# robotseu/ORB_Line_SLAM

Measured on AMD Instinct MI355X. Metric: stereo frames/s extract+match (ORB+LBD), KITTI 1242x375, higher is better.
Workload: dtype u8; 1 GPU; C3: 1242x375 stereo, 2000 ORB + 500 LBD per image, extract + stereo point/line match + f2f LBD match + SearchByBoW vs the previous frame (synthetic k=10 L=6 vocabulary, ComputeBoW included); parallelism=frame-sharded x1, distinct_pairs=512, order=shuffled, scene=default

## Files before the change

orb_line_slam_amd/csrc/api.cpp:

```cpp
#include "olf_internal.hpp"
#include "line_internal.hpp"
#include "../../include/orbline.h"
#include <map>
#include <mutex>
#include <cstring>
#include <mutex>

namespace olf {
static thread_local std::string g_err;
void set_error(const std::string& s) { g_err = s; }
}

using namespace olf;

struct olf_ctx {
    olf_params params;
    int W = 0, H = 0, max_images = 0;
    int device = 0;
    hipStream_t stream = nullptr;
    OrbHostTables orb;
    OrbDeviceBufs ob;
    uint8_t* d_images = nullptr;
    olf_keypoint* d_kps = nullptr;
    uint8_t* d_desc = nullptr;
// ... 183 lines not shown
    for (void* p : c->allocs) (void)hipFree(p);
    for (void* p : c->scratch) if (p) (void)hipFree(p);
    for (auto& r : c->prof_recs) { (void)hipEventDestroy(r.a); (void)hipEventDestroy(r.b); }
    for (hipEvent_t e : c->prof_pool) (void)hipEventDestroy(e);
    if (c->ev_fork) (void)hipEventDestroy(c->ev_fork);
    if (c->ev_front) (void)hipEventDestroy(c->ev_front);
    if (c->ev_sort) (void)hipEventDestroy(c->ev_sort);
    if (c->ev_lbd) (void)hipEventDestroy(c->ev_lbd);
    if (c->ev_join) (void)hipEventDestroy(c->ev_join);
    if (c->stream2) (void)hipStreamDestroy(c->stream2);
    if (c->stream) (void)hipStreamDestroy(c->stream);
    delete c;
}

int olf_ctx_create(const olf_params* p, int width, int height, int max_images, olf_ctx** out)
{
    if (!p || !out || width < 64 || height < 64 || max_images < 1) { set_error("olf_ctx_create: bad argument"); return OLF_ERR_INVALID; }
    *out = nullptr;
    if (p->abi_version != OLF_ABI_VERSION || p->struct_size != (uint32_t)sizeof(olf_params)) {
        set_error("olf_ctx_create: the parameter block was not initialised by this library's olf_default_params() (abi_version / struct_size differ: "
                  "caller built against another include/orbline_types.h)");
        return OLF_ERR_INVALID;
    }
    int ndev = 0;
    if (hipGetDeviceCount(&ndev) != hipSuccess || ndev < 1) {
        set_error("olf_ctx_create: no HIP device visible (this library has no CPU path)");
        return OLF_ERR_NODEVICE;
    }
    olf_ctx* c = new olf_ctx();
    c->params = *p; c->W = width; c->H = height; c->max_images = max_images;
    int rc = c->orb.build(p->orb, width, height);
    if (rc != OLF_OK) {
        set_error(rc == OLF_ERR_CAPACITY ? "olf_ctx_create: more than 32760 key points on one pyramid level (nfeatures too large for this scale factor / level count)"
                                         : "olf_ctx_create: image size / ORB parameters not supported (every pyramid level needs at least 62 x 62 pixels and a landscape cell grid)");
        delete c; return rc;
    }
    auto fail = [&](int code) { olf_ctx_destroy(c); return code; };
    if (hipGetDevice(&c->device) != hipSuccess) return fail(OLF_ERR_HIP);
    if (hipDeviceGetAttribute(&c->limits.nCU, hipDeviceAttributeMultiprocessorCount, c->device) != hipSuccess || c->limits.nCU <= 0) c->limits.nCU = 64;
    if (hipDeviceGetAttribute(&c->limits.maxLds, hipDeviceAttributeMaxSharedMemoryPerBlock, c->device) != hipSuccess) c->limits.maxLds = 64 * 1024;
    if (hipStreamCreateWithFlags(&c->stream, hipStreamNonBlocking) != hipSuccess) { set_error("hipStreamCreate failed"); return fail(OLF_ERR_HIP); }
    const OrbGeom& g = c->orb.geom;
    const size_t n = (size_t)max_images;
    OrbDeviceBufs& b = c->ob;
    const bool allocTrace = getenv("OLF_ALLOC_TRACE") != nullptr;
#define A(ptr, count) do { if ((rc = dev_alloc(c, &(ptr), (count))) != OLF_OK) return fail(rc); \
                           if (allocTrace) fprintf(stderr, "alloc %-18s %8.3f MB per image\n", #ptr, (double)(count) * sizeof(*(ptr)) / 1e6 / (double)n); } while (0)
    A(b.pyr, n * g.pyrBytes); A(b.blur, n * g.pyrBytes);
    A(b.cells, n * g.totalCells * g.cellCap); A(b.cellCount, n * g.totalCells);
    A(b.cand, n * g.candTotal); A(b.candNode, n * g.candTotal); A(b.candCount, n * g.nlevels);
    if (g.maxNodes > 2048) A(b.octSpill, n * g.nlevels * octree_lds_bytes(g.maxNodes));
    A(b.lvlKp, n * g.kpTotal); A(b.lvlCount, n * g.nlevels); A(b.lvlAngle, n * g.kpTotal);
    A(b.rx, c->orb.rx.size() + 1); A(b.ry, c->orb.ry.size() + 1); A(b.geom, 1); A(b.status, 256);
    A(c->d_uright, ((n + 1) / 2) * g.outCap); A(c->d_depth, ((n + 1) / 2) * g.outCap); A(c->d_sad, ((n + 1) / 2) * g.outCap); A(c->d_bestkey, ((n + 1) / 2) * g.outCap); A(c->d_rowperm, n * g.outCap);
    A(c->d_images, n * width * height); A(c->d_kps, n * g.outCap); A(c->d_desc, n * g.outCap * OLF_DESC_BYTES); A(c->d_counts, n);
#undef A
    if (hipMemcpy(b.rx, c->orb.rx.data(), c->orb.rx.size() * sizeof(ResizeCoef), hipMemcpyHostToDevice) != hipSuccess ||
        hipMemcpy(b.ry, c->orb.ry.data(), c->orb.ry.size() * sizeof(ResizeCoef), hipMemcpyHostToDevice) != hipSuccess ||
        hipMemcpy(b.geom, &g, sizeof(OrbGeom), hipMemcpyHostToDevice) != hipSuccess ||
        hipMemset(b.status, 0, 1024) != hipSuccess) {
        set_error("olf_ctx_create: table upload failed");
        return fail(OLF_ERR_HIP);
    }
    rc = c->line.build(p->line, width, height, max_images);
    if (rc != OLF_OK) { set_error("olf_ctx_create: LSD parameters not supported"); return fail(rc); }
    LineGeom& lg = c->line.geom;
    int prLeast = 0, prGreatest = 0;
    (void)hipDeviceGetStreamPriorityRange(&prLeast, &prGreatest);
    if (hipStreamCreateWithPriority(&c->stream2, hipStreamNonBlocking, prLeast) != hipSuccess ||
        hipEventCreateWithFlags(&c->ev_fork, hipEventDisableTiming) != hipSuccess || hipEventCreateWithFlags(&c->ev_front, hipEventDisableTiming) != hipSuccess || hipEventCreateWithFlags(&c->ev_sort, hipEventDisableTiming) != hipSuccess ||
        hipEventCreateWithFlags(&c->ev_lbd, hipEventDisableTiming) != hipSuccess ||
        hipEventCreateWithFlags(&c->ev_join, hipEventDisableTiming) != hipSuccess) { set_error("stream/event creation failed"); return fail(OLF_ERR_HIP); }
    LineDeviceBufs& l = c->lb;
#define A(ptr, count) do { if ((rc = dev_alloc(c, &(ptr), (count))) != OLF_OK) return fail(rc); \
                           if (allocTrace) fprintf(stderr, "alloc %-18s %8.3f MB per image\n", #ptr, (double)(count) * sizeof(*(ptr)) / 1e6 / (double)n); } while (0)
    const bool batchCtx = n > (size_t)kBatchCtxImages;
    const size_t keyWords = lg.wide ? 2 : 1;
    A(l.grad, n * lg.Ps); A(l.keysA, n * lg.Ps * keyWords); A(l.keysB, n * lg.Ps * keyWords);
    if (batchCtx && lg.Ps * 4 >= lg.pitchW * lg.H && lg.Ps * 4 >= lg.pitchS * lg.Hs) { l.lsdBlur = reinterpret_cast<uint8_t*>(l.keysA); l.scaled = reinterpret_cast<uint8_t*>(l.keysB); c->scaled_aliased = true; }
    else { A(l.lsdBlur, n * lg.pitchW * lg.H); A(l.scaled, n * lg.pitchS * lg.Hs); }
    A(l.topBuf, n * (size_t)lsd_seedsort_top_words()); A(l.keyCount, n * 32); A(l.maxN, n * 32); A(l.chunkCnt, n * ((lg.Ps + 4095) / 4096)); A(l.sortHist, n * (size_t)lsd_sort_max_chunks(lg.Ps) * 32); A(l.sortBase, n * 32);
    l.nChunks = lg.regionStride / 32;
    A(l.region, n * (size_t)lg.regionStride); l.ownerImages = (batchCtx || lg.wide) ? 0 : (int)std::min<size_t>(n, kMwMaxImages); A(l.owner, (size_t)l.ownerImages * lg.Ps); A(l.links, n * (size_t)l.nChunks);
    lg.logCap = lg.regionStride / 2;
    lg.spillBlocks = lg.regionStride / 2 >= lg.Ps ? 0 : (int)std::max<size_t>(4, n / 16);
    if (lg.spillBlocks) A(lg.spillArena, (size_t)lg.spillBlocks * 2 * lg.Ps);
    A(lg.spillCtl, 64); A(lg.spillOf, n);
    l.mgImages = (int)std::min<size_t>(n, kMgMaxImages); l.mgStride = lsd_grow_mg_stride(lg.maxRegions);
    A(l.mg, (size_t)l.mgImages * l.mgStride);
    A(l.rawLines, n * lg.maxDetect); A(l.rawCount, n); A(l.regCount, n); A(l.growFmt, n); A(l.lbdBlur, n * lg.pitchW * lg.H); A(l.dxdy, n * lg.pitchD * lg.H);
    A(l.rowSums, n * lg.outCap * 63 * 4); A(l.lbdStarts, n * lg.outCap * 64 * 2); A(l.rx, c->line.rx.size()); A(l.ry, c->line.ry.size()); A(l.geom, 1);
    A(c->d_kls, n * lg.outCap); A(c->d_ldesc, n * lg.outCap * OLF_DESC_BYTES); A(c->d_lcounts, n);
    {
        const size_t np = (n + 1) / 2;
        A(c->d_ldist, np * lg.outCap * lg.outCap); A(c->d_lm21, np * lg.outCap); A(c->d_lm12, np * lg.outCap);
        A(c->d_ldisp, np * lg.outCap * 2); A(c->d_lle, np * lg.outCap * 3);
        void* q = nullptr;
        if (hipMalloc(&q, stereo_lines_prep_bytes((int)n, lg.outCap)) != hipSuccess) { set_error("hipMalloc failed"); return fail(OLF_ERR_HIP); }
        c->allocs.push_back(q); c->d_lprep = q;
    }
    if (n <= 16) {
        const size_t np = (n + 1) / 2, ocap = g.outCap, lcap = lg.outCap;
        const size_t sz[11] = {n * ocap * sizeof(olf_keypoint), n * ocap * OLF_DESC_BYTES, n * sizeof(int), np * ocap * sizeof(float), np * ocap * sizeof(float),
                               n * lcap * sizeof(olf_keyline), n * lcap * OLF_DESC_BYTES, n * sizeof(int), np * lcap * sizeof(int), np * lcap * 2 * sizeof(float), np * lcap * 3 * sizeof(double)};
        size_t off = 0;
        for (int k = 0; k < 11; ++k) { c->outslab_off[k] = off; off += (sz[k] + 255) & ~(size_t)255; }
        c->outslab_off[11] = off; c->outslab_bytes = off;
        A(c->d_outslab, off);
        if (hipHostMalloc(reinterpret_cast<void**>(&c->h_outslab), off, hipHostMallocDefault) != hipSuccess) { set_error("hipHostMalloc failed"); return fail(OLF_ERR_HIP); }
        uint8_t* q = c->d_outslab;
        c->d_kps = reinterpret_cast<olf_keypoint*>(q + c->outslab_off[0]); c->d_desc = q + c->outslab_off[1]; c->d_counts = reinterpret_cast<int*>(q + c->outslab_off[2]);
        c->d_uright = reinterpret_cast<float*>(q + c->outslab_off[3]); c->d_depth = reinterpret_cast<float*>(q + c->outslab_off[4]);
// ... 882 lines not shown
```

orb_line_slam_amd/csrc/filters.hip:

```cpp
#include "olf_internal.hpp"
#include <algorithm>

namespace olf {

constexpr int SF_TW = 128, SF_TH = 32;
constexpr int SF_INW = (SF_TW + 8) / 4;
constexpr int SF_INH = SF_TH + 6;

__device__ __forceinline__ int sf_reflect(int p, int n)
{
    if (p < 0) p = -p;
    if (p >= n) p = 2 * (n - 1) - p;
    return p;
}

__global__ __launch_bounds__(256) void k_sep7(const uint8_t* __restrict__ src, size_t srcImgStride, int srcPitch, uint8_t* __restrict__ dst,
                                              size_t dstImgStride, int dstPitch, int W, int H, Taps7 taps)
{
    __shared__ uint32_t s_in[SF_INH * SF_INW];
    constexpr int HS = (SF_INH + 1) / 2 + ((((SF_INH + 1) / 2) & 1) ? 0 : 1);
    __shared__ uint32_t s_h[SF_TW * HS];
    const int img = blockIdx.z, x0 = blockIdx.x * SF_TW, y0 = blockIdx.y * SF_TH;
    const uint8_t* s = src + (size_t)img * srcImgStride;
    const bool plain = x0 >= 4 && x0 + SF_TW + 4 <= W && y0 >= 3 && y0 + SF_TH + 3 <= H && ((srcPitch | (int)srcImgStride) & 3) == 0 &&
// ... 53 lines not shown
        const uint32_t D0 = hp[0], D1 = hp[1], D2 = hp[2], D3 = hp[3], D4 = hp[4];
        const uint32_t E0 = __builtin_amdgcn_alignbyte(D1, D0, 2u), E1 = __builtin_amdgcn_alignbyte(D2, D1, 2u);
        const uint32_t E2 = __builtin_amdgcn_alignbyte(D3, D2, 2u), E3 = __builtin_amdgcn_alignbyte(D4, D3, 2u);
        res[0][c] = dot2(D3, t6lo, dot2(D2, t45, dot2(D1, t23, dot2(D0, t01, 32768u))));
        res[1][c] = dot2(D3, t6hi, dot2(E2, t45, dot2(E1, t23, dot2(E0, t01, 32768u))));
        res[2][c] = dot2(D4, t6lo, dot2(D3, t45, dot2(D2, t23, dot2(D1, t01, 32768u))));
        res[3][c] = dot2(D4, t6hi, dot2(E3, t45, dot2(E2, t23, dot2(E1, t01, 32768u))));
    }
    uint8_t* d = dst + (size_t)img * dstImgStride;
#pragma unroll
    for (int rr = 0; rr < 4; ++rr) {
        const int gy = y0 + ry0 + rr;
        if (gy >= H) break;
        const uint32_t a0 = min(res[rr][0] >> 16, 255u), a1 = min(res[rr][1] >> 16, 255u), a2 = min(res[rr][2] >> 16, 255u), a3 = min(res[rr][3] >> 16, 255u);
        uint8_t* o = d + (size_t)gy * dstPitch + gx;
        if (gx + 3 < W && ((reinterpret_cast<uintptr_t>(o) & 3) == 0))
            *reinterpret_cast<uint32_t*>(o) = a0 | (a1 << 8) | (a2 << 16) | (a3 << 24);
        else {
            o[0] = (uint8_t)a0;
            if (gx + 1 < W) o[1] = (uint8_t)a1;
            if (gx + 2 < W) o[2] = (uint8_t)a2;
            if (gx + 3 < W) o[3] = (uint8_t)a3;
        }
    }
}

constexpr int SS_ROWS = 16;
constexpr int SS_BROWS = 8;

__device__ __forceinline__ int ss_reflect(int p, int n) { p = p < 0 ? -p : p; return p >= n ? 2 * (n - 1) - p : p; }

template <bool BORDER, int ROWS>
__device__ __forceinline__ void sep7_strip_body(const int t, const uint8_t* __restrict__ src, size_t srcImgStride, int srcPitch, uint8_t* __restrict__ dst,
                                                size_t dstImgStride, int dstPitch, int W, int H, const Taps7& taps, int nsx, int nsy)
{
    const int nb = BORDER ? 1 + ((W + 3) / 4 - (nsx + 1)) : nsx;
    if (t >= nb * nsy) return;
    const int sy = t / nb, si = t - sy * nb;
    const int sx = BORDER ? (si == 0 ? 0 : nsx + si) : si + 1;
    const int x0 = 4 * sx, y0 = sy * ROWS;
    const uint8_t* s = src + (size_t)blockIdx.y * srcImgStride + (x0 - 4);
    uint8_t* d = dst + (size_t)blockIdx.y * dstImgStride + x0;
    const uint32_t tlo = (uint32_t)taps.t[0] | ((uint32_t)taps.t[1] << 8) | ((uint32_t)taps.t[2] << 16) | ((uint32_t)taps.t[3] << 24);
    const uint32_t thi = (uint32_t)taps.t[4] | ((uint32_t)taps.t[5] << 8) | ((uint32_t)taps.t[6] << 16);
    const uint32_t t01 = (uint32_t)taps.t[0] | ((uint32_t)taps.t[1] << 16), t23 = (uint32_t)taps.t[2] | ((uint32_t)taps.t[3] << 16);
    const uint32_t t45 = (uint32_t)taps.t[4] | ((uint32_t)taps.t[5] << 16), t6lo = (uint32_t)taps.t[6], t6hi = (uint32_t)taps.t[6] << 16;
    typedef unsigned short us2 __attribute__((ext_vector_type(2)));
    auto dot2 = [](uint32_t a, uint32_t b, uint32_t c) -> uint32_t {
        us2 va, vb;
        __builtin_memcpy(&va, &a, 4); __builtin_memcpy(&vb, &b, 4);
        return __builtin_amdgcn_udot2(va, vb, c, false);
    };
    struct Raw { uint32_t w[3]; };
    auto load_row = [&](int y) -> Raw {
        Raw r;
        const uint8_t* row = s + (size_t)ss_reflect(min(y, H + 2), H) * srcPitch;
        if (!BORDER) __builtin_memcpy(r.w, row, 12);
        else {
#pragma unroll
            for (int k = 0; k < 3; ++k) {
                uint32_t v = 0;
#pragma unroll
                for (int b = 0; b < 4; ++b) {
                    const int x = x0 - 4 + 4 * k + b;
                    v |= (uint32_t)row[ss_reflect(min(x, W + 2), W) - (x0 - 4)] << (8 * b);
                }
                r.w[k] = v;
            }
        }
        return r;
    };
    auto hrow = [&](const Raw& r, uint32_t* o) {
        const uint32_t* w = r.w;
        o[0] = __builtin_amdgcn_udot4(__builtin_amdgcn_alignbyte(w[2], w[1], 1u), thi, __builtin_amdgcn_udot4(__builtin_amdgcn_alignbyte(w[1], w[0], 1u), tlo, 0u, false), false);
        o[1] = __builtin_amdgcn_udot4(__builtin_amdgcn_alignbyte(w[2], w[1], 2u), thi, __builtin_amdgcn_udot4(__builtin_amdgcn_alignbyte(w[1], w[0], 2u), tlo, 0u, false), false);
        o[2] = __builtin_amdgcn_udot4(__builtin_amdgcn_alignbyte(w[2], w[1], 3u), thi, __builtin_amdgcn_udot4(__builtin_amdgcn_alignbyte(w[1], w[0], 3u), tlo, 0u, false), false);
        o[3] = __builtin_amdgcn_udot4(w[2], thi, __builtin_amdgcn_udot4(w[1], tlo, 0u, false), false);
    };
    auto pair = [&](const Raw& ra, const Raw& rb, uint32_t* Pj) {
        uint32_t a[4], b[4];
        hrow(ra, a); hrow(rb, b);
#pragma unroll
        for (int c = 0; c < 4; ++c) Pj[c] = a[c] | (b[c] << 16);
    };
    uint32_t P[ROWS / 2 + 3][4];
    Raw nx[4];
    {
        Raw r0 = load_row(y0 - 3), r1 = load_row(y0 - 2), r2 = load_row(y0 - 1), r3 = load_row(y0), r4 = load_row(y0 + 1), r5 = load_row(y0 + 2);
#pragma unroll
        for (int k = 0; k < 4; ++k) nx[k] = load_row(y0 + 3 + k);
        pair(r0, r1, P[0]); pair(r2, r3, P[1]); pair(r4, r5, P[2]);
    }
#pragma unroll
    for (int g = 0; g < ROWS / 4; ++g) {
        const Raw c0 = nx[0], c1 = nx[1], c2 = nx[2], c3 = nx[3];
        if (g + 1 < ROWS / 4) {
#pragma unroll
            for (int k = 0; k < 4; ++k) nx[k] = load_row(y0 + 4 * (g + 1) + 3 + k);
            __builtin_amdgcn_sched_barrier(0);
        }
        pair(c0, c1, P[2 * g + 3]); pair(c2, c3, P[2 * g + 4]);
        uint32_t res[4][4];
#pragma unroll
        for (int c = 0; c < 4; ++c) {
            const uint32_t D0 = P[2 * g][c], D1 = P[2 * g + 1][c], D2 = P[2 * g + 2][c], D3 = P[2 * g + 3][c], D4 = P[2 * g + 4][c];
            const uint32_t E0 = __builtin_amdgcn_alignbyte(D1, D0, 2u), E1 = __builtin_amdgcn_alignbyte(D2, D1, 2u);
            const uint32_t E2 = __builtin_amdgcn_alignbyte(D3, D2, 2u), E3 = __builtin_amdgcn_alignbyte(D4, D3, 2u);
            res[0][c] = dot2(D3, t6lo, dot2(D2, t45, dot2(D1, t23, dot2(D0, t01, 32768u))));
            res[1][c] = dot2(D3, t6hi, dot2(E2, t45, dot2(E1, t23, dot2(E0, t01, 32768u))));
            res[2][c] = dot2(D4, t6lo, dot2(D3, t45, dot2(D2, t23, dot2(D1, t01, 32768u))));
            res[3][c] = dot2(D4, t6hi, dot2(E3, t45, dot2(E2, t23, dot2(E1, t01, 32768u))));
        }
#pragma unroll
        for (int rr = 0; rr < 4; ++rr) {
            const int gy = y0 + 4 * g + rr;
            if (gy < H) {
                const uint32_t a0 = min(res[rr][0] >> 16, 255u), a1 = min(res[rr][1] >> 16, 255u), a2 = min(res[rr][2] >> 16, 255u), a3 = min(res[rr][3] >> 16, 255u);
                const uint32_t v = a0 | (a1 << 8) | (a2 << 16) | (a3 << 24);
                if (!BORDER) __builtin_memcpy(d + (size_t)gy * dstPitch, &v, 4);
                else {
#pragma unroll
                    for (int b = 0; b < 4; ++b) if (x0 + b < W) d[(size_t)gy * dstPitch + b] = (uint8_t)(v >> (8 * b));
                }
            }
        }
    }
}

template <bool BORDER>
__global__ __launch_bounds__(256) void k_sep7_strip(const uint8_t* __restrict__ src, size_t srcImgStride, int srcPitch, uint8_t* __restrict__ dst,
                                                    size_t dstImgStride, int dstPitch, int W, int H, Taps7 taps, int nsx, int nsy)
{
    sep7_strip_body<BORDER, BORDER ? SS_BROWS : SS_ROWS>(blockIdx.x * 256 + threadIdx.x, src, srcImgStride, srcPitch, dst, dstImgStride, dstPitch, W, H, taps, nsx, nsy);
}
// ... 248 lines not shown
```

orb_line_slam_amd/csrc/host_tables.cpp:

```cpp
#include "olf_internal.hpp"
#include "line_internal.hpp"
#include <algorithm>
#include <cmath>
#include <cfenv>

namespace olf {

static inline int cv_round_f(float v) { return (int)lrintf(v); }
static inline int cv_round_d(double v) { return (int)lrint(v); }
static inline int cv_floor(double v) { int i = (int)v; return i - (i > v); }
static inline int cv_ceil(double v) { int i = (int)v; return i + (i < v); }

std::vector<int> gaussian_taps_q8(int n, double sigma, int sum256)
{
    if (sum256) {
        std::vector<double> k(n);
        double s = 0;
        const double scale2X = -0.5 / (sigma * sigma);
        for (int i = 0; i < n; ++i) { const double x = i - (n - 1) * 0.5; k[i] = std::exp(scale2X * x * x); s += k[i]; }
        std::vector<int> q(n);
        double err = 0;
        int sum = 0;
        for (int i = 0; i < n / 2; ++i) {
            const double adj = k[i] / s * 256.0 + err;
// ... 85 lines not shown
        int v, v0, vmax = cv_floor(kHalfPatch * std::sqrt(2.f) / 2 + 1);
        int vmin = cv_ceil(kHalfPatch * std::sqrt(2.f) / 2);
        const double hp2 = kHalfPatch * kHalfPatch;
        for (v = 0; v <= vmax; ++v) g.umax[v] = cv_round_d(std::sqrt(hp2 - v * v));
        for (v = kHalfPatch, v0 = 0; v >= vmin; --v) {
            while (g.umax[v0] == g.umax[v0 + 1]) ++v0;
            g.umax[v] = v0;
            ++v0;
        }
    }
    std::vector<int> taps = gaussian_taps_q8(7, 2.0, p.conv_gauss_sum256);
    for (int i = 0; i < 7; ++i) g.blurTaps[i] = taps[i];

    rx.clear(); ry.clear();
    int off = 0, cells = 0, cand = 0, kps = 0, cellCap = 1, maxQuota = 1, maxKp = 1;
    for (int l = 0; l < nlevels; ++l) {
        LevelGeom& L = g.lv[l];
        L.w = cv_round_f((float)W * inv_sf[l]);
        L.h = cv_round_f((float)H * inv_sf[l]);
        if (L.w - 2 * kMinBorder < 30 || L.h - 2 * kMinBorder < 30) return OLF_ERR_INVALID;
        L.pitch = (L.w + 63) & ~63;
        L.offset = off;
        off += L.pitch * L.h;
        off = (off + 255) & ~255;
        L.maxBorderX = L.w - kMinBorder; L.maxBorderY = L.h - kMinBorder;
        const float width = (float)(L.maxBorderX - kMinBorder), height = (float)(L.maxBorderY - kMinBorder);
        L.nCols = (int)(width / 30.f); L.nRows = (int)(height / 30.f);
        L.wCell = (int)std::ceil(width / L.nCols); L.hCell = (int)std::ceil(height / L.nRows);
        L.wCellM = (uint32_t)(((1u << 20) + L.wCell - 1) / L.wCell); L.hCellM = (uint32_t)(((1u << 20) + L.hCell - 1) / L.hCell);
        if (L.w >= (1 << 14) || L.h >= (1 << 14) || L.wCell > 64 || L.hCell > 64) { L.wCellM = 0; L.hCellM = 0; }
        L.cellBase = cells;
        cells += L.nCols * L.nRows;
        cellCap = std::max(cellCap, ((L.wCell + 1) / 2) * ((L.hCell + 1) / 2));
        L.quota = nPerLevel[l];
        maxQuota = std::max(maxQuota, L.quota);
        L.nIni = (int)std::round(width / height);
        if (L.nIni < 1) return OLF_ERR_INVALID;
        L.hX = width / L.nIni;
        L.scale = sf[l]; L.inv_scale = inv_sf[l];
        L.patch_size = (int)(31 * sf[l]);
        L.kpBase = kps; L.kpCap = std::max(L.quota + 8, 4 * L.nIni + 4); kps += L.kpCap;
        maxKp = std::max(maxKp, L.kpCap);
        if (l > 0) {
            const LevelGeom& P = g.lv[l - 1];
            L.resizeTabX = (int)rx.size(); L.resizeTabY = (int)ry.size();
            rx.resize(rx.size() + L.w); ry.resize(ry.size() + L.h);
            double inv_x = (double)L.w / P.w, inv_y = (double)L.h / P.h;
            resize_axis_coefs(P.w, L.w, 1. / inv_x, true, &rx[L.resizeTabX]);
            resize_axis_coefs(P.h, L.h, 1. / inv_y, false, &ry[L.resizeTabY]);
            L.resizeTiled = resize_tiled_fits(&rx[L.resizeTabX], &ry[L.resizeTabY], P.w, P.h, L.w, L.h) ? 1 : 0;
            if (L.resizeTiled && resize_strip_fits(&rx[L.resizeTabX], P.w, L.w)) L.resizeTiled |= 2;
        }
    }
    g.pyrBytes = off;
    g.totalCells = cells;
    g.cellCap = cellCap;
    if (cellCap > 1024) return OLF_ERR_CAPACITY;
    for (int l = 0; l < nlevels; ++l) {
        LevelGeom& L = g.lv[l];
        long cap = (long)L.nCols * L.nRows * cellCap;
        L.candCap = (int)std::min<long>(cap, 65535);
        L.candBase = cand;
        cand += (L.candCap + 63) & ~63;
    }
    g.candTotal = cand;
    g.kpTotal = kps;
    g.outCap = kps;
    int mn = 64;
    while (mn < maxKp) mn <<= 1;
    g.maxNodes = mn;
    if (mn > 32768) return OLF_ERR_CAPACITY;
    return OLF_OK;
}

int LineHostTables::build(const olf_line_params& p, int W, int H, int max_images)
{
    LineGeom& g = geom;
    g = LineGeom();
    if (p.lsd_refine < 0 || p.lsd_refine > 2) return OLF_ERR_INVALID;
    if (p.conv_seed_order != 0 && p.conv_seed_order != 1) return OLF_ERR_INVALID;
    if (p.conv_libm_float != 0 && p.conv_libm_float != 1) return OLF_ERR_INVALID;
    if (!(p.lsd_scale > 0) || p.lsd_n_bins < 2 || p.lsd_n_bins > (1 << 24) || !(p.lsd_ang_th > 0 && p.lsd_ang_th < 180)) return OLF_ERR_INVALID;
    const double kPI = 3.1415926535897932384626433832795;
    g.W = W; g.H = H; g.pitchW = (W + 63) & ~63; g.pitchD = (W + 3) & ~3;
    g.scale = p.lsd_scale;
    g.Ws = cv_round_d(W * p.lsd_scale); g.Hs = cv_round_d(H * p.lsd_scale);
    g.pitchS = (g.Ws + 63) & ~63;
    g.Ps = g.Ws * g.Hs;
    {
        int k = 0; while ((1 << k) < g.Ws) ++k;
        const int p = std::max(32, 22 + k);
        const unsigned long long M = ((1ull << p) + (unsigned long long)g.Ws - 1) / (unsigned long long)g.Ws;
        g.divWsM = (uint32_t)M; g.divWsS = p - 32;
    }
    g.libmFloat = p.conv_libm_float ? 1 : 0;
    g.alignDeg = p.lsd_ang_th < 90 ? (float)(180.0 - p.lsd_ang_th) : -1.f;
    g.regionStride = std::max(1024 + g.Ps / 32 + 64, (2 * g.Ps + 31) / 32) * 32;
    if (max_images > kBatchCtxImages) g.regionStride = ((std::max(g.Ps, 8192) + 31) / 32) * 32;
    if ((long)g.Ws * g.Hs >= (1L << 27) || g.Ws < 8 || g.Hs < 8 || g.Ws > 32767 || g.Hs > 32767) return OLF_ERR_INVALID;
    g.wide = (p.lsd_n_bins > 1024 || (long)g.Ws * g.Hs >= (1L << 22)) ? 1 : 0;
    g.prec = kPI * p.lsd_ang_th / 180;
    {
        const long double w = (long double)(2 * kPI) - (long double)g.prec;
        double t = (double)w;
        if ((long double)t < w) t = std::nextafter(t, 1e300);
        g.precWrap = t;
// ... 72 lines not shown
```

orb_line_slam_amd/csrc/olf_internal.hpp:

```cpp
#pragma once
#include <hip/hip_runtime.h>
#include <stdint.h>
#include <string>
#include <vector>
#include "../../include/orbline_types.h"

#define OLF_HIP_CHECK(expr)                                                                 \
    do {                                                                                    \
        hipError_t _e = (expr);                                                             \
        if (_e != hipSuccess) {                                                             \
            olf::set_error(std::string(#expr) + ": " + hipGetErrorString(_e));              \
            return OLF_ERR_HIP;                                                             \
        }                                                                                   \
    } while (0)

namespace olf {

void set_error(const std::string& s);

#ifdef __HIPCC__
__device__ __forceinline__ int wave_sum_i32(int v)
{
    v += __builtin_amdgcn_mov_dpp(v, 0xB1, 0xf, 0xf, true);
    v += __builtin_amdgcn_mov_dpp(v, 0x4E, 0xf, 0xf, true);
    v += __builtin_amdgcn_mov_dpp(v, 0x141, 0xf, 0xf, true);
    v += __builtin_amdgcn_mov_dpp(v, 0x140, 0xf, 0xf, true);
    return __builtin_amdgcn_readlane(v, 0) + __builtin_amdgcn_readlane(v, 16) + __builtin_amdgcn_readlane(v, 32) + __builtin_amdgcn_readlane(v, 48);
}

__device__ __forceinline__ int wave_min_i32(int v)
{
    v = min(v, __builtin_amdgcn_update_dpp(v, v, 0xB1, 0xf, 0xf, false));
    v = min(v, __builtin_amdgcn_update_dpp(v, v, 0x4E, 0xf, 0xf, false));
    v = min(v, __builtin_amdgcn_update_dpp(v, v, 0x141, 0xf, 0xf, false));
    v = min(v, __builtin_amdgcn_update_dpp(v, v, 0x140, 0xf, 0xf, false));
    return min(min(__builtin_amdgcn_readlane(v, 0), __builtin_amdgcn_readlane(v, 16)), min(__builtin_amdgcn_readlane(v, 32), __builtin_amdgcn_readlane(v, 48)));
}
__device__ __forceinline__ unsigned long long wave_vote(bool p) { return __builtin_amdgcn_ballot_w64(p); }
__device__ __forceinline__ int wave_rank_below(unsigned long long m) { return (int)__builtin_amdgcn_mbcnt_hi((unsigned)(m >> 32), __builtin_amdgcn_mbcnt_lo((unsigned)m, 0u)); }
__device__ __forceinline__ bool wave_bit(unsigned long long m) { return __builtin_amdgcn_inverse_ballot_w64(m); }
#endif

constexpr int kEdge = 19;
constexpr int kMinBorder = 16;
constexpr int kHalfPatch = 15;

struct LevelGeom {
    int w, h, pitch;
    int offset;
    int maxBorderX, maxBorderY;
    int nCols, nRows, wCell, hCell;
    uint32_t wCellM, hCellM;
    int cellBase;
    int quota;
    int nIni;
    float hX;
    float scale;
    float inv_scale;
    int patch_size;
    int candBase;
    int candCap;
    int kpBase, kpCap;
    int resizeTabX, resizeTabY;
    int resizeTiled;
};

struct ResizeCoef { int16_t ofs; int16_t a0; int16_t a1; int16_t pad; };

struct OrbGeom {
    int nlevels;
    int W, H, in_pitch;
    int pyrBytes;
    int totalCells;
    int cellCap;
    int candTotal;
    int kpTotal;
    int outCap;
    int iniTh, minTh;
    int maxNodes;
    LevelGeom lv[OLF_MAX_LEVELS];
    int umax[16];
    int blurTaps[7];
};

struct OrbHostTables {
    std::vector<float> sf, inv_sf, sigma2, inv_sigma2;
    std::vector<int> nPerLevel;
    OrbGeom geom;
    std::vector<ResizeCoef> rx, ry;
    int build(const olf_orb_params& p, int W, int H);
};

std::vector<int> gaussian_taps_q8(int n, double sigma, int sum256 = 0);
void resize_axis_coefs(int sn, int dn, double scale, bool clamp_like_x, ResizeCoef* coef);

struct OrbDeviceBufs {
    uint8_t* pyr = nullptr;
    uint8_t* blur = nullptr;
    uint32_t* cells = nullptr;
    int* cellCount = nullptr;
    uint32_t* cand = nullptr;
    uint16_t* candNode = nullptr;
    int* candCount = nullptr;
    uint32_t* lvlKp = nullptr;
    int* lvlCount = nullptr;
    float* lvlAngle = nullptr;
    ResizeCoef* rx = nullptr;
    ResizeCoef* ry = nullptr;
    OrbGeom* geom = nullptr;
    int* status = nullptr;
    unsigned char* octSpill = nullptr;
};

int launch_orb_pyramid(const OrbGeom& g, const OrbDeviceBufs& b, const uint8_t* d_in, int n_images, hipStream_t s);
int launch_orb_fast(const OrbGeom& g, const OrbDeviceBufs& b, int n_images, hipStream_t s);
int launch_orb_octree(const OrbGeom& g, const OrbDeviceBufs& b, int n_images, hipStream_t s);
size_t octree_lds_bytes(int M);
int launch_orb_blur(const OrbGeom& g, const OrbDeviceBufs& b, int n_images, hipStream_t s);
int launch_orb_describe(const OrbGeom& g, const OrbDeviceBufs& b, int n_images, olf_keypoint* d_kps, uint8_t* d_desc,
                        int* d_counts, int out_cap, hipStream_t s);

struct Taps7 { int t[7]; };
int launch_sep7(const uint8_t* src, size_t srcImgStride, int srcPitch, uint8_t* dst, size_t dstImgStride, int dstPitch, int W, int H,
                const int* taps7, int n_images, hipStream_t s);
int launch_sep_wide(const uint8_t* src, size_t srcImgStride, int srcPitch, uint8_t* dst, size_t dstImgStride, int dstPitch, int W, int H,
                    const int* taps, int r, int n_images, hipStream_t s);

bool resize_tiled_fits(const ResizeCoef* rx, const ResizeCoef* ry, int sw, int sh, int dw, int dh);
bool resize_strip_fits(const ResizeCoef* rx, int sw, int dw, int ncols = 4);
int launch_resize_tiled(const uint8_t* src, size_t srcImgStride, int srcPitch, int sw, int sh, uint8_t* dst, size_t dstImgStride, int dstPitch,
                        int dw, int dh, const ResizeCoef* d_rx, const ResizeCoef* d_ry, int n_images, hipStream_t s, bool strip = false);

int launch_cvt_gray(const uint8_t* src, uint8_t* dst, int w, int h, int code, int n_images, hipStream_t s);
int launch_init_rectify_map(const double* ir9, const double* k8, double fx, double fy, double u0, double v0, int w, int h, float* d_map1, float* d_map2,
                            hipStream_t s);
int launch_remap_linear(const uint8_t* src, int sw, int sh, const float* mapx, const float* mapy, int dw, int dh, uint8_t* dst, int n_images,
                        hipStream_t s);

int launch_stereo_points(const OrbGeom& g, const OrbDeviceBufs& b, int n_pairs, const olf_keypoint* d_kps, const uint8_t* d_desc,
                         const int* d_counts, int cap, float mbf, float fx, float* d_uRight, float* d_depth, int* d_sad, int* d_bestKey,
                         unsigned* d_perm, hipStream_t s);
int launch_match_bf(const uint8_t* dA, const int* nA, int strideA, int aStep, const uint8_t* dB, const int* nB, int strideB, int bStep,
                    int n_sets, float nnr, int best_lr, int* ws, int* m12, hipStream_t s);
int launch_knn2(const uint8_t* dA, const int* nA, int strideA, const uint8_t* dB, const int* nB, int strideB, int n_sets, int* idx0,
                int* dist0, int* dist1, hipStream_t s);
int launch_match_candidates(const uint8_t* q, int nQ, const uint8_t* t, int nT, const int* offs, const int* cand, uint16_t* out, hipStream_t s);
int launch_distinctive(const uint8_t* desc, const int* offs, int n_points, int* best, hipStream_t s);
int launch_hamming_matrix(const uint8_t* a, int nA, const uint8_t* b, int nB, uint16_t* out, hipStream_t s);

}
```

orb_line_slam_amd/csrc/orb_pyramid.hip:

```cpp
#include "olf_internal.hpp"

namespace olf {

__global__ __launch_bounds__(256) void k_ingest(const uint8_t* __restrict__ in, uint8_t* __restrict__ pyr,
                                                int W, int H, int in_pitch, int pitch0, int pyrBytes)
{
    const int img = blockIdx.y;
    const int segs = (W + 15) >> 4;
    const int idx = blockIdx.x * 256 + threadIdx.x;
    if (idx >= segs * H) return;
    const int y = idx / segs, x = (idx - y * segs) * 16;
    const uint8_t* src = in + (size_t)img * H * in_pitch + (size_t)y * in_pitch + x;
    uint4 v = make_uint4(0u, 0u, 0u, 0u);
    if (x + 16 <= W) __builtin_memcpy(&v, src, 16);
    else {
        uint32_t w[4] = {0u, 0u, 0u, 0u};
#pragma unroll
        for (int k = 0; k < 16; ++k)
            if (x + k < W) w[k >> 2] |= (uint32_t)src[k] << (8 * (k & 3));
        v = make_uint4(w[0], w[1], w[2], w[3]);
    }
    *reinterpret_cast<uint4*>(pyr + (size_t)img * pyrBytes + (size_t)y * pitch0 + x) = v;
}

__global__ __launch_bounds__(256) void k_resize(uint8_t* __restrict__ pyr, int pyrBytes, LevelGeom P, LevelGeom L,
                                                const ResizeCoef* __restrict__ rx, const ResizeCoef* __restrict__ ry)
{
    const int img = blockIdx.y;
    const int quads = (L.w + 3) >> 2;
    const int idx = blockIdx.x * 256 + threadIdx.x;
    if (idx >= quads * L.h) return;
    const int dy = idx / quads, dx0 = (idx - dy * quads) * 4;
    const uint8_t* src = pyr + (size_t)img * pyrBytes + P.offset;
    const ResizeCoef cy = ry[L.resizeTabY + dy];
    const int y0 = min(max((int)cy.ofs, 0), P.h - 1), y1 = min(max((int)cy.ofs + 1, 0), P.h - 1);
    const uint8_t* S0 = src + (size_t)y0 * P.pitch;
    const uint8_t* S1 = src + (size_t)y1 * P.pitch;
    const int b0 = cy.a0, b1 = cy.a1;
    uint32_t out = 0;
#pragma unroll
    for (int k = 0; k < 4; ++k) {
        const int dx = dx0 + k;
        if (dx < L.w) {
            const ResizeCoef cx = rx[L.resizeTabX + dx];
            const int sx = cx.ofs, sx1 = min(sx + 1, P.w - 1);
            const int h0 = S0[sx] * cx.a0 + S0[sx1] * cx.a1;
            const int h1 = S1[sx] * cx.a0 + S1[sx1] * cx.a1;
            const int v = (((b0 * (h0 >> 4)) >> 16) + ((b1 * (h1 >> 4)) >> 16) + 2) >> 2;
            out |= (uint32_t)(v & 0xff) << (8 * k);
        }
    }
    *reinterpret_cast<uint32_t*>(pyr + (size_t)img * pyrBytes + L.offset + (size_t)dy * L.pitch + dx0) = out;
}

constexpr int FT_W = 128;
constexpr int FT_EW = 124;
constexpr int FT_INW = (FT_W + 8) / 4;


template <int NT>
__global__ __launch_bounds__(NT) __attribute__((amdgpu_waves_per_eu(8, 8)))
void k_fast_score(const uint8_t* __restrict__ pyr, int pyrBytes, LevelGeom L, int minTh,
                  uint32_t* __restrict__ cells, int* __restrict__ cellCount, int totalCells, int cellCap)
{
    constexpr int FT_H = NT / 8, FT_EH = FT_H - 2, FT_INH = FT_H + 6;
    __shared__ uint32_t tile[FT_INH * FT_INW];
    __shared__ unsigned short s_cand[FT_W * FT_H];
    unsigned short* const s_list = s_cand;
    __shared__ uint8_t s_score[FT_H * FT_W];
    __shared__ int s_nc, s_n;
    const int img = blockIdx.z;
    const int x0 = kMinBorder - 4 + blockIdx.x * FT_EW, y0 = kMinBorder + 2 + blockIdx.y * FT_EH;
    const int xBeg = kMinBorder + 3, yBeg = kMinBorder + 3, xEnd = L.maxBorderX - 3, yEnd = L.maxBorderY - 3;
    const uint8_t* src = pyr + (size_t)img * pyrBytes + L.offset;
    {
        constexpr int NLD = (FT_INH * FT_INW + NT - 1) / NT;
        uint32_t tv[NLD];
#pragma unroll
        for (int k = 0; k < NLD; ++k) {
            const int i = threadIdx.x + k * NT;
            const int r = i / FT_INW, j = i - r * FT_INW;
            const int gy = min(y0 - 3 + r, L.h - 1);
            const int xw = min(x0 - 4 + 4 * j, L.pitch - 4);
            tv[k] = i < FT_INH * FT_INW ? *reinterpret_cast<const uint32_t*>(src + (size_t)gy * L.pitch + xw) : 0u;
        }
#pragma unroll
        for (int k = 0; k < NLD; ++k) { const int i = threadIdx.x + k * NT; if (i < FT_INH * FT_INW) tile[i] = tv[k]; }
    }
    reinterpret_cast<uint4*>(s_score)[threadIdx.x] = make_uint4(0u, 0u, 0u, 0u);
    if (threadIdx.x == 0) { s_nc = 0; s_n = 0; }
    __syncthreads();
    const int q = threadIdx.x & 31, ry0 = (threadIdx.x >> 5) * 4;
    uint32_t w[10][3];
#pragma unroll
    for (int r = 0; r < 10; ++r)
#pragma unroll
        for (int k = 0; k < 3; ++k) w[r][k] = tile[(ry0 + r) * FT_INW + q + k];
    uint32_t hE[10], hO[10];
#pragma unroll
    for (int r = 0; r < 10; ++r) {
        hE[r] = __builtin_amdgcn_perm(w[r][1], w[r][1], 0x0c020c00u);
        hO[r] = __builtin_amdgcn_perm(w[r][1], w[r][1], 0x0c030c01u);
    }
    const uint32_t K = 0x02000200u - (uint32_t)(minTh + 1) * 0x00010001u, C9 = 0x02000200u;
    uint32_t acc = 0;
#pragma unroll
    for (int rr = 0; rr < 4; ++rr) {
        const int c = rr + 3;
        const uint32_t eE = __builtin_amdgcn_perm(w[c][2], w[c][1], 0x0c050c03u), eO = __builtin_amdgcn_perm(w[c][2], w[c][1], 0x0c060c04u);
        const uint32_t wE = __builtin_amdgcn_perm(w[c][1], w[c][0], 0x0c030c01u), wO = __builtin_amdgcn_perm(w[c][1], w[c][0], 0x0c040c02u);
        uint32_t ps[2];
#pragma unroll
        for (int h = 0; h < 2; ++h) {
            const uint32_t V = h ? hO[c] : hE[c], N8 = h ? hO[c - 3] : hE[c - 3], N0 = h ? hO[c + 3] : hE[c + 3], N4 = h ? eO : eE, N12 = h ? wO : wE;
            const uint32_t Bb = K - V, Bd = V + K;
            const uint32_t br = ((N0 + Bb) | (N8 + Bb)) & ((N4 + Bb) | (N12 + Bb));
            const uint32_t dk = ((Bd - N0) | (Bd - N8)) & ((Bd - N4) | (Bd - N12));
            ps[h] = br | dk;
        }
        acc = (acc >> 2) | (ps[0] & C9) | ((ps[1] << 1) & (C9 << 1));
    }
    acc >>= 3;
    {
        uint32_t cols = 0, bm = 0;
#pragma unroll
// ... 128 lines not shown
    int kept = n;
    if (anyIni) {
        int drop = 0;
        for (int i = lane; i < n; i += 64)
            if ((int)(s_k[i] & 0xffu) < g.iniTh) { s_k[i] = 0xffffffffu; ++drop; }
#pragma unroll
        for (int o = 32; o > 0; o >>= 1) drop += __shfl_xor(drop, o);
        kept = n - drop;
        __builtin_amdgcn_wave_barrier();
    }
    for (int k = 2; k <= sortN; k <<= 1)
        for (int j = k >> 1; j > 0; j >>= 1) {
            for (int t = lane; t < sortN; t += 64) {
                const int p = t ^ j;
                if (p > t) {
                    const uint32_t a = s_k[t], b = s_k[p];
                    if (((t & k) == 0) ? a > b : a < b) { s_k[t] = b; s_k[p] = a; }
                }
            }
            __builtin_amdgcn_wave_barrier();
        }
    for (int i = lane; i < kept; i += 64) {
        const uint32_t k = s_k[i];
        slot[i] = (((k >> 8) & 0xfffu) << 20) | ((k >> 20) << 8) | (k & 0xffu);
    }
    if (lane == 0) *cnt = kept;
}

int launch_orb_pyramid(const OrbGeom& g, const OrbDeviceBufs& b, const uint8_t* d_in, int n_images, hipStream_t s)
{
    {
        const int quads = ((g.W + 15) >> 4) * g.H;
        hipLaunchKernelGGL(k_ingest, dim3((quads + 255) / 256, n_images), dim3(256), 0, s, d_in, b.pyr, g.W, g.H, g.in_pitch,
                           g.lv[0].pitch, g.pyrBytes);
    }
    for (int l = 1; l < g.nlevels; ++l) {
        const LevelGeom &P = g.lv[l - 1], &L = g.lv[l];
        if (L.resizeTiled) {
            int rc = launch_resize_tiled(b.pyr + P.offset, (size_t)g.pyrBytes, P.pitch, P.w, P.h, b.pyr + L.offset, (size_t)g.pyrBytes, L.pitch, L.w, L.h,
                                         b.rx + L.resizeTabX, b.ry + L.resizeTabY, n_images, s, (L.resizeTiled & 2) != 0);
            if (rc != OLF_OK) return rc;
        } else {
            const int quads = ((L.w + 3) >> 2) * L.h;
            hipLaunchKernelGGL(k_resize, dim3((quads + 255) / 256, n_images), dim3(256), 0, s, b.pyr, g.pyrBytes, P, L, b.rx, b.ry);
        }
    }
    OLF_HIP_CHECK(hipGetLastError());
    return OLF_OK;
}

int launch_orb_fast(const OrbGeom& g, const OrbDeviceBufs& b, int n_images, hipStream_t s)
{
    OLF_HIP_CHECK(hipMemsetAsync(b.cellCount, 0, (size_t)n_images * g.totalCells * sizeof(int), s));
    for (int l = 0; l < g.nlevels; ++l) {
        const LevelGeom& L = g.lv[l];
        const int fw = L.maxBorderX - 3 - (kMinBorder - 2), fh = L.maxBorderY - 3 - (kMinBorder + 3);
        if (fw <= 0 || fh <= 0) continue;
        hipLaunchKernelGGL(k_fast_score<256>, dim3((fw + FT_EW - 1) / FT_EW, (fh + 30 - 1) / 30, n_images), dim3(256), 0, s, b.pyr,
                           g.pyrBytes, L, g.minTh, b.cells, b.cellCount, g.totalCells, g.cellCap);
    }
    hipLaunchKernelGGL(k_cells_sort, dim3(g.totalCells, n_images), dim3(64), 0, s, b.geom, b.cells, b.cellCount);
    OLF_HIP_CHECK(hipGetLastError());
    return OLF_OK;
}

int launch_orb_blur(const OrbGeom& g, const OrbDeviceBufs& b, int n_images, hipStream_t s)
{
    for (int l = 0; l < g.nlevels; ++l) {
        const LevelGeom& L = g.lv[l];
        int rc = launch_sep7(b.pyr + L.offset, (size_t)g.pyrBytes, L.pitch, b.blur + L.offset, (size_t)g.pyrBytes, L.pitch, L.w, L.h, g.blurTaps,
                             n_images, s);
        if (rc != OLF_OK) return rc;
    }
    return OLF_OK;
}

}
```

Before: 15100 stereo frames/s.

## Merge per-level FAST launches into one tile-table kernel; vectorize border blur loads

The per-pyramid-level FAST scoring launches are replaced by a single launch. It indexes a precomputed device table of (level, tileY, tileX) entries and reads level geometry from device memory. This removes several kernel launches per frame batch and lets small levels share the GPU, at the cost of an extra table read per block. Separately, the border path of the separable blur now does one 12-byte load and reflects pixels with byte-permute selectors instead of per-byte gathers.

```diff
diff --git a/orb_line_slam_amd/csrc/api.cpp b/orb_line_slam_amd/csrc/api.cpp
--- a/orb_line_slam_amd/csrc/api.cpp
+++ b/orb_line_slam_amd/csrc/api.cpp
@@ -259,12 +259,14 @@
     if (g.maxNodes > 2048) A(b.octSpill, n * g.nlevels * octree_lds_bytes(g.maxNodes));
     A(b.lvlKp, n * g.kpTotal); A(b.lvlCount, n * g.nlevels); A(b.lvlAngle, n * g.kpTotal);
     A(b.rx, c->orb.rx.size() + 1); A(b.ry, c->orb.ry.size() + 1); A(b.geom, 1); A(b.status, 256);
+    b.nFastTiles = (int)c->orb.fastTiles.size(); A(b.fastTiles, c->orb.fastTiles.size() + 1);
     A(c->d_uright, ((n + 1) / 2) * g.outCap); A(c->d_depth, ((n + 1) / 2) * g.outCap); A(c->d_sad, ((n + 1) / 2) * g.outCap); A(c->d_bestkey, ((n + 1) / 2) * g.outCap); A(c->d_rowperm, n * g.outCap);
     A(c->d_images, n * width * height); A(c->d_kps, n * g.outCap); A(c->d_desc, n * g.outCap * OLF_DESC_BYTES); A(c->d_counts, n);
 #undef A
     if (hipMemcpy(b.rx, c->orb.rx.data(), c->orb.rx.size() * sizeof(ResizeCoef), hipMemcpyHostToDevice) != hipSuccess ||
         hipMemcpy(b.ry, c->orb.ry.data(), c->orb.ry.size() * sizeof(ResizeCoef), hipMemcpyHostToDevice) != hipSuccess ||
         hipMemcpy(b.geom, &g, sizeof(OrbGeom), hipMemcpyHostToDevice) != hipSuccess ||
+        hipMemcpy(b.fastTiles, c->orb.fastTiles.data(), c->orb.fastTiles.size() * sizeof(uint32_t), hipMemcpyHostToDevice) != hipSuccess ||
         hipMemset(b.status, 0, 1024) != hipSuccess) {
         set_error("olf_ctx_create: table upload failed");
         return fail(OLF_ERR_HIP);
diff --git a/orb_line_slam_amd/csrc/filters.hip b/orb_line_slam_amd/csrc/filters.hip
--- a/orb_line_slam_amd/csrc/filters.hip
+++ b/orb_line_slam_amd/csrc/filters.hip
@@ -129,23 +129,32 @@
         return __builtin_amdgcn_udot2(va, vb, c, false);
     };
     struct Raw { uint32_t w[3]; };
+    const int xa = BORDER ? max(0, min(x0 - 4, W - 12)) : x0 - 4;
+    uint32_t selLo[3] = {0, 0, 0}, selHi[3] = {0, 0, 0};
+    if (BORDER) {
+#pragma unroll
+        for (int k = 0; k < 3; ++k)
+#pragma unroll
+            for (int b = 0; b < 4; ++b) {
+                const int x = x0 - 4 + 4 * k + b;
+                const uint32_t i = (uint32_t)(ss_reflect(min(x, W + 2), W) - xa);
+                selLo[k] |= (i < 8u ? i : 0x0cu) << (8 * b);
+                selHi[k] |= (i < 8u ? 0x0cu : i - 8u) << (8 * b);
+            }
+    }
     auto load_row = [&](int y) -> Raw {
         Raw r;
         const uint8_t* row = s + (size_t)ss_reflect(min(y, H + 2), H) * srcPitch;
         if (!BORDER) __builtin_memcpy(r.w, row, 12);
-        else {
-#pragma unroll
-            for (int k = 0; k < 3; ++k) {
-                uint32_t v = 0;
-#pragma unroll
-                for (int b = 0; b < 4; ++b) {
-                    const int x = x0 - 4 + 4 * k + b;
-                    v |= (uint32_t)row[ss_reflect(min(x, W + 2), W) - (x0 - 4)] << (8 * b);
-                }
-                r.w[k] = v;
-            }
-        }
+        else __builtin_memcpy(r.w, row + (xa - (x0 - 4)), 12);
         return r;
+    };
+    auto window = [&](const Raw& r) -> Raw {
+        if (!BORDER) return r;
+        Raw o;
+#pragma unroll
+        for (int k = 0; k < 3; ++k) o.w[k] = __builtin_amdgcn_perm(r.w[1], r.w[0], selLo[k]) | __builtin_amdgcn_perm(r.w[2], r.w[2], selHi[k]);
+        return o;
     };
     auto hrow = [&](const Raw& r, uint32_t* o) {
         const uint32_t* w = r.w;
@@ -156,7 +165,7 @@
     };
     auto pair = [&](const Raw& ra, const Raw& rb, uint32_t* Pj) {
         uint32_t a[4], b[4];
-        hrow(ra, a); hrow(rb, b);
+        hrow(window(ra), a); hrow(window(rb), b);
 #pragma unroll
         for (int c = 0; c < 4; ++c) Pj[c] = a[c] | (b[c] << 16);
     };
diff --git a/orb_line_slam_amd/csrc/host_tables.cpp b/orb_line_slam_amd/csrc/host_tables.cpp
--- a/orb_line_slam_amd/csrc/host_tables.cpp
+++ b/orb_line_slam_amd/csrc/host_tables.cpp
@@ -161,6 +161,16 @@
             if (L.resizeTiled && resize_strip_fits(&rx[L.resizeTabX], P.w, L.w)) L.resizeTiled |= 2;
         }
     }
+    fastTiles.clear();
+    for (int l = 0; l < nlevels; ++l) {
+        const LevelGeom& L = g.lv[l];
+        const int fw = L.maxBorderX - 3 - (kMinBorder - 2), fh = L.maxBorderY - 3 - (kMinBorder + 3);
+        if (fw <= 0 || fh <= 0) continue;
+        const int nx = (fw + kFastTileW - 1) / kFastTileW, ny = (fh + kFastTileH - 1) / kFastTileH;
+        if (nx > 4096 || ny > 4096) return OLF_ERR_INVALID;
+        for (int ty = 0; ty < ny; ++ty)
+            for (int tx = 0; tx < nx; ++tx) fastTiles.push_back((uint32_t)l << 24 | (uint32_t)ty << 12 | (uint32_t)tx);
+    }
     g.pyrBytes = off;
     g.totalCells = cells;
     g.cellCap = cellCap;
diff --git a/orb_line_slam_amd/csrc/olf_internal.hpp b/orb_line_slam_amd/csrc/olf_internal.hpp
--- a/orb_line_slam_amd/csrc/olf_internal.hpp
+++ b/orb_line_slam_amd/csrc/olf_internal.hpp
@@ -44,6 +44,7 @@
 constexpr int kEdge = 19;
 constexpr int kMinBorder = 16;
 constexpr int kHalfPatch = 15;
+constexpr int kFastTileW = 124, kFastTileH = 30;
 
 struct LevelGeom {
     int w, h, pitch;
@@ -88,6 +89,7 @@
     std::vector<int> nPerLevel;
     OrbGeom geom;
     std::vector<ResizeCoef> rx, ry;
+    std::vector<uint32_t> fastTiles;
     int build(const olf_orb_params& p, int W, int H);
 };
 
@@ -108,6 +110,8 @@
     ResizeCoef* rx = nullptr;
     ResizeCoef* ry = nullptr;
     OrbGeom* geom = nullptr;
+    uint32_t* fastTiles = nullptr;
+    int nFastTiles = 0;
     int* status = nullptr;
     unsigned char* octSpill = nullptr;
 };
diff --git a/orb_line_slam_amd/csrc/orb_pyramid.hip b/orb_line_slam_amd/csrc/orb_pyramid.hip
--- a/orb_line_slam_amd/csrc/orb_pyramid.hip
+++ b/orb_line_slam_amd/csrc/orb_pyramid.hip
@@ -54,23 +54,27 @@
 }
 
 constexpr int FT_W = 128;
-constexpr int FT_EW = 124;
+constexpr int FT_EW = kFastTileW;
 constexpr int FT_INW = (FT_W + 8) / 4;
 
 
 template <int NT>
 __global__ __launch_bounds__(NT) __attribute__((amdgpu_waves_per_eu(8, 8)))
-void k_fast_score(const uint8_t* __restrict__ pyr, int pyrBytes, LevelGeom L, int minTh,
+void k_fast_score(const uint8_t* __restrict__ pyr, int pyrBytes, const OrbGeom* __restrict__ gp, const uint32_t* __restrict__ tiles, int minTh,
                   uint32_t* __restrict__ cells, int* __restrict__ cellCount, int totalCells, int cellCap)
 {
     constexpr int FT_H = NT / 8, FT_EH = FT_H - 2, FT_INH = FT_H + 6;
+    static_assert(FT_EH == kFastTileH, "the tile table is built for this tile");
+    const uint32_t te = tiles[blockIdx.x];
+    const LevelGeom& L = gp->lv[te >> 24];
+    const int tileX = (int)(te & 0xfffu), tileY = (int)((te >> 12) & 0xfffu);
     __shared__ uint32_t tile[FT_INH * FT_INW];
     __shared__ unsigned short s_cand[FT_W * FT_H];
     unsigned short* const s_list = s_cand;
     __shared__ uint8_t s_score[FT_H * FT_W];
     __shared__ int s_nc, s_n;
-    const int img = blockIdx.z;
-    const int x0 = kMinBorder - 4 + blockIdx.x * FT_EW, y0 = kMinBorder + 2 + blockIdx.y * FT_EH;
+    const int img = blockIdx.y;
+    const int x0 = kMinBorder - 4 + tileX * FT_EW, y0 = kMinBorder + 2 + tileY * FT_EH;
     const int xBeg = kMinBorder + 3, yBeg = kMinBorder + 3, xEnd = L.maxBorderX - 3, yEnd = L.maxBorderY - 3;
     const uint8_t* src = pyr + (size_t)img * pyrBytes + L.offset;
     {
@@ -305,13 +309,9 @@
 int launch_orb_fast(const OrbGeom& g, const OrbDeviceBufs& b, int n_images, hipStream_t s)
 {
     OLF_HIP_CHECK(hipMemsetAsync(b.cellCount, 0, (size_t)n_images * g.totalCells * sizeof(int), s));
-    for (int l = 0; l < g.nlevels; ++l) {
-        const LevelGeom& L = g.lv[l];
-        const int fw = L.maxBorderX - 3 - (kMinBorder - 2), fh = L.maxBorderY - 3 - (kMinBorder + 3);
-        if (fw <= 0 || fh <= 0) continue;
-        hipLaunchKernelGGL(k_fast_score<256>, dim3((fw + FT_EW - 1) / FT_EW, (fh + 30 - 1) / 30, n_images), dim3(256), 0, s, b.pyr,
-                           g.pyrBytes, L, g.minTh, b.cells, b.cellCount, g.totalCells, g.cellCap);
-    }
+    if (b.nFastTiles > 0)
+        hipLaunchKernelGGL(k_fast_score<256>, dim3(b.nFastTiles, n_images), dim3(256), 0, s, b.pyr, g.pyrBytes, b.geom, b.fastTiles, g.minTh, b.cells, b.cellCount,
+                           g.totalCells, g.cellCap);
     hipLaunchKernelGGL(k_cells_sort, dim3(g.totalCells, n_images), dim3(64), 0, s, b.geom, b.cells, b.cellCount);
     OLF_HIP_CHECK(hipGetLastError());
     return OLF_OK;
```

New measurement: 15160 stereo frames/s, median of 6. Within noise of the previous version (+0.4%).
